# QingzhiWang/LIS-SLAM

Measured on AMD Instinct MI355X. Metric: scan-to-submap registrations/sec (64x1800 pts, 200k submap), higher is better.
Workload: dtype f32; 1 GPU; configs[1]: batch=64 synthetic 64x1800 scans vs one shared 200k-pt submap per GPU, semantic mask off, 10 fixed GN iterations, target index build inside the step; batch_per_gpu=64, submap_points=200000, gn_iters=10, parallelism=independent batches x1 + RCCL all-gather of results

## Files before the change

### lis-slam_amd/csrc/lisreg_api_batch.hip

```cpp
#include "lisreg_batch_plan.hpp"

#include <algorithm>
#include <chrono>
#include <cmath>
#include <cstdio>
#include <cstdlib>
#include <cstring>
#include <string>
#include <vector>

using namespace lisreg;

namespace {

struct CtxTargets {
    const std::vector<Target>& v;
    size_t size() const { return v.size(); }
    TargetView operator()(int slot) const
    {
        const Target& t = v[(size_t)slot];
        return TargetView{ t.valid, { t.n[0], t.n[1] }, { t.n_cells[0], t.n_cells[1] }, { &t.g[0], &t.g[1] }, { t.raw_ptr[0], t.raw_ptr[1] },
                           { t.sorted[0].as<float4>(), t.sorted[1].as<float4>() }, { t.cell_start[0].as<int>(), t.cell_start[1].as<int>() } };
    }
};
// ... 301 lines not shown
    ctx_prof_mark(c, -1);
    return LISREG_OK;
}

void dispatch_order_tables(lisreg_ctx* c, Split split, hipStream_t st)
{
    const auto [o, b] = view(c);
    if (!c->last.xcd_now || (b.live.xcd_cached && split.blk == 0)) return;
    const float4* sorted = b.sort_now ? c->sorted_all.as<float4>() : nullptr;
    const bool by_target = many_targets(o, b);
    int* const pos = c->xcd_tab.as<int>();
    int* const ids = pos + b.n_blocks;
    const int nb0 = split.blk ? split.blk : b.n_blocks;
    launch_xcd_order(c->blocks.as<BlockDesc>(), nb0, c->segs.as<Segment>(), c->grids_dev.as<GridIndex>(), c->items.as<ItemState>(),
                     sorted, by_target, pos, ids, st);
    if (!split.blk) return;
    launch_xcd_order(c->blocks.as<BlockDesc>() + split.blk, b.n_blocks - split.blk, c->segs.as<Segment>(), c->grids_dev.as<GridIndex>(),
                     c->items.as<ItemState>(), sorted, by_target, pos + split.blk, ids + split.blk, st);
    c->batch.live.xcd_cached = false;
}

struct RunHalf { int i0, ni, b0, nb; hipStream_t s; int sidx; hipEvent_t after_assoc; };

void iteration(lisreg_ctx* c, const DevParams& prm, int it, const RunHalf& h)
{
    const auto [o, b] = view(c);
    if (!h.after_assoc) ctx_prof_mark(c, 0, h.sidx);
    (o.exact ? launch_assoc_exact : launch_assoc)(
                 c->blocks.as<BlockDesc>() + h.b0, h.nb, c->segs.as<Segment>(), c->grids_dev.as<GridIndex>(),
                 c->items.as<ItemState>(), prm, b.sort_now ? c->sorted_all.as<float4>() : nullptr, c->partials.as<double>() + (size_t)h.b0 * kNumAcc,
                 b.mode_now, c->nn.as<int>(), b.n_elems, o.first_pass_r * o.first_pass_r,
                 b.mode_now != 5 && it >= (b.lanes_q == 8 ? kWideFromSmall : kWideFrom) && it <= (b.mode_now == 3 ? kGraphWideUntil : kWideUntil), kGraphHops,
                 o.count_searches ? c->counters.as<unsigned long long>() : nullptr,
                 o.dump_neighbors ? c->dbg_nn.as<int>() : nullptr, b.lanes_q,
                 c->blocks_q.as<BlockDesc>(), (int)b.h_blocks_q.size(), c->coef.as<float4>(), c->coef_ok.as<int>(),
                 c->last.xcd_now ? c->xcd_tab.as<int>() + b.n_blocks + h.b0 : nullptr, h.s);
    if (h.after_assoc) (void)hipEventRecord(h.after_assoc, h.s);
    ctx_prof_mark(c, 1, h.sidx);
    launch_solve(c->items.as<ItemState>() + h.i0, h.ni, prm, c->partials.as<double>(),
                 o.trace_cap > 0 ? c->trace.as<float>() + (size_t)h.i0 * (size_t)o.trace_cap * kTraceStride : nullptr, o.trace_cap, c->done_dev.as<int>(), h.s);
    ctx_prof_mark(c, -1, h.sidx);
}

int run_plain(lisreg_ctx* c, const DevParams& prm, bool can_stop, hipStream_t st)
{
    const auto [o, b] = view(c);
    const int chunk = o.early_stop_chunk > 0 ? o.early_stop_chunk : (b.n_blocks <= 1024 ? 6 : 3);
    int next_check = chunk;
    if (o.early_stop_chunk <= 0 && c->mem.last_launches > 0) next_check = std::max(2, std::min(c->mem.last_launches, chunk));
    const RunHalf all{ 0, b.n_items, 0, b.n_blocks, st, 0, nullptr };
    for (int it = 0; it < prm.bound; ++it) {
        iteration(c, prm, it, all);
        if (o.exact && it + 1 < prm.bound) { int rc = exact_pose_caches(c); if (rc) return rc; }
        if (can_stop && it + 1 == next_check && it + 1 < prm.bound) {
            HIPCHK(c, hipMemcpyAsync(c->done_host.p, c->done_dev.p, sizeof(int), hipMemcpyDeviceToHost, st));
            HIPCHK(c, hipStreamSynchronize(st));
            if (*c->done_host.as<int>() >= b.n_items) break;
            next_check += o.early_stop_chunk > 0 ? chunk : std::min(chunk, 3);
        }
    }
    return LISREG_OK;
}

int run_interleaved(lisreg_ctx* c, const DevParams& prm, Split split, hipStream_t st)
{
    const auto [o, b] = view(c);
    c->last.interleaved_now = true;
    const bool alternate = o.interleave == 1 && c->ev_ab && c->ev_ba;
    const RunHalf A{ 0, split.item, 0, split.blk, st, 0, alternate ? (hipEvent_t)c->ev_ab : nullptr };
    const RunHalf B{ split.item, b.n_items - split.item, split.blk, b.n_blocks - split.blk, c->side_stream, 1, alternate ? (hipEvent_t)c->ev_ba : nullptr };
    hipError_t ie = hipSuccess;
    for (int it = 0; it < prm.bound && ie == hipSuccess; ++it) {
        if (alternate && it > 0) ie = hipStreamWaitEvent(st, c->ev_ba, 0);
        if (ie != hipSuccess) break;
        if (alternate) ctx_prof_mark(c, 0, 0);
        iteration(c, prm, it, A);
        if (alternate) ie = hipStreamWaitEvent(c->side_stream, c->ev_ab, 0);
        if (ie != hipSuccess) break;
        if (alternate) ctx_prof_mark(c, 0, 1);
        iteration(c, prm, it, B);
    }
    if (ie == hipSuccess) ie = hipEventRecord(c->ev_join, c->side_stream);
    if (ie == hipSuccess) ie = hipStreamWaitEvent(st, c->ev_join, 0);
    if (ie == hipSuccess) return LISREG_OK;
    (void)hipStreamSynchronize(c->side_stream);
    c->last.interleaved_now = false;
    return ctx_fail(c, LISREG_ERR_HIP, std::string("interleaved run: ") + hipGetErrorString(ie));
}

int finalize_run(lisreg_ctx* c, const DevParams& prm, hipStream_t st)
{
    launch_finalize(c->items.as<ItemState>(), c->batch.n_items, prm, c->results.as<float>(), st, c->done_dev.as<int>());
    c->batch.live.items_reset = true; ++c->batch.live.runs_since_fetch;
    HIPCHK(c, hipGetLastError());
    if (c->pack_in_use >= 0 && c->pack_free[c->pack_in_use])
        HIPCHK(c, hipEventRecord(c->pack_free[c->pack_in_use], st));
    return LISREG_OK;
}

int run_impl(lisreg_ctx* c, bool early_stop)
{
    if (!c->batch.live.prepared) return bad(c, "batch_run: no prepared batch");
    HIPCHK(c, hipSetDevice(c->device));
    const auto [o, b] = view(c);
    PreparedBatch::Live& live = c->batch.live;
    hipStream_t st = c->stream;
    c->last.xcd_now = xcd_order_wanted(o, b);
    if (c->last.xcd_now) HIPCHK(c, c->xcd_tab.ensure(sizeof(int) * 2 * (size_t)b.n_blocks));
    const bool can_stop = early_stop && b.prm.fixed_iters <= 0 && c->done_host.p && o.early_stop_chunk != 0;
    const Split split = choose_split(c, can_stop);
    c->last.reach_now = o.rebuild_targets_each_run && b.mode_now == 5 && live.reach_ready && !o.exact;
    DevParams prm = b.prm;
    prm.reach_miss = c->last.reach_now ? reach_miss_counter(c) : nullptr;
    const bool reset_done = live.items_reset;
    live.items_reset = false;
    if (o.rebuild_targets_each_run) { int rc = rebuild_targets(c, st); if (rc) return rc; }
    if (!reset_done) launch_reset_items(c->items.as<ItemState>(), b.n_items, prm, c->done_dev.as<int>(), st);
    if (o.exact) { int rc = exact_pose_caches(c); if (rc) return rc; }
    ctx_prof_mark(c, 2);
    launch_sort_sources(c->blocks.as<BlockDesc>(), b.n_blocks, c->segs.as<Segment>(), b.n_segs, c->items.as<ItemState>(),
                        b.n_elems, b.sort_now ? b.n_buckets : 0, sort_buffers(c), c->sorted_all.as<float4>(), c->order_all.as<int>(), st);
    ctx_prof_mark(c, -1);
    dispatch_order_tables(c, split, st);
    prm.cell_anchor_until = o.cell_anchor_until;
    c->last.interleaved_now = false;
    int rc;
    if (split.blk > 0 && hipEventRecord(c->ev_fork, st) == hipSuccess && hipStreamWaitEvent(c->side_stream, c->ev_fork, 0) == hipSuccess)
        rc = run_interleaved(c, prm, split, st);
    else
        rc = run_plain(c, prm, can_stop, st);
    return rc ? rc : finalize_run(c, prm, st);
}

using HostClock = std::chrono::steady_clock;
int prepare_run_fetch(lisreg_ctx* c, int n_items, const lisreg_item* dev_items, const lisreg_params* params, float* T, lisreg_stats* stats,
                      const HostClock::time_point* prof)
{
    int rc = lisreg_batch_prepare(c, n_items, dev_items, params, T);
    if (rc) { (void)hipStreamSynchronize(c->stream); return rc; }
    const auto t1 = prof ? HostClock::now() : HostClock::time_point();
    rc = run_impl(c, true);
    if (rc) { (void)hipStreamSynchronize(c->stream); return rc; }
    const auto t2 = prof ? HostClock::now() : HostClock::time_point();
    rc = lisreg_batch_fetch(c, T, stats);
    if (prof) {
        auto us = [](auto a, auto b) { return std::chrono::duration<double, std::micro>(b - a).count(); };
        fprintf(stderr, "[lisreg host] upload %.1f us, prepare %.1f us, enqueue %.1f us, fetch (incl. GPU wait) %.1f us\n",
                us(prof[0], prof[1]), us(prof[1], t1), us(t1, t2), us(t2, HostClock::now()));
    }
    return rc;
}

}

// ... 177 lines not shown
```

### lis-slam_amd/csrc/lisreg_api_ctx.hip

```cpp
#include "lisreg_ctx.hpp"

#include <algorithm>
#include <cmath>
#include <cstring>
#include <string>
#include <vector>

namespace lisreg {

static thread_local std::string g_static_err;
int ctx_fail(lisreg_ctx* c, int code, const std::string& msg)
{
    if (c) c->err = msg; else g_static_err = msg;
    return code;
}

int bad(lisreg_ctx* c, const std::string& msg) { return ctx_fail(c, LISREG_ERR_ARG, msg); }

int check_cloud(lisreg_ctx* c, const char* who, const void* cloud, int n, int stride, int fmt, unsigned accepted_formats, bool allow_empty)
{
    if (n < 0 || (n == 0 && !allow_empty)) return bad(c, std::string(who) + (allow_empty ? ": n < 0" : ": n <= 0"));
    if (n > 0 && !cloud) return bad(c, std::string(who) + ": NULL cloud with n > 0");
    if (fmt < 0 || fmt >= 32 || !(accepted_formats & fmt_bit(fmt))) return bad(c, std::string(who) + ": this fmt is not accepted here");
    if (fmt_bit(fmt) & kFmtDevice) return LISREG_OK;
// ... 115 lines not shown
void make_grid(const float bb_in[6], int n, GridIndex* g, int* n_cells, int margin_cells)
{
    float bb[6] = { bb_in[0], bb_in[1], bb_in[2], bb_in[3], bb_in[4], bb_in[5] };
    memset(g, 0, sizeof *g);
    g->n = n;
    float cell = 0.5f;
    if (n > 0) {
        const double area = std::max(1.0, (double)(bb[3] - bb[0]) * (double)(bb[4] - bb[1]));
        cell = (float)std::min(0.5, std::max(0.25, 2.8 / std::sqrt((double)n / area)));
    }
    if (n <= 0) { g->cell = cell; g->inv_cell = 1.f / cell; g->nx = g->ny = g->nz = 0; *n_cells = 1; return; }
    const double max_cells = 1 << 24;
    const float bb0[6] = { bb[0], bb[1], bb[2], bb[3], bb[4], bb[5] };
    for (;;) {
        for (int d = 0; d < 3; ++d) { bb[d] = bb0[d] - (float)margin_cells * cell; bb[3 + d] = bb0[3 + d] + (float)margin_cells * cell; }
        double nx = floor((bb[3] - bb[0]) / cell) + 1, ny = floor((bb[4] - bb[1]) / cell) + 1,
               nz = floor((bb[5] - bb[2]) / cell) + 1;
        if (nx * ny * nz <= max_cells) { g->nx = (int)nx; g->ny = (int)ny; g->nz = (int)nz; break; }
        cell *= 1.26f;
    }
    g->ox = bb[0]; g->oy = bb[1]; g->oz = bb[2];
    g->cell = cell; g->inv_cell = 1.f / cell;
    *n_cells = g->nx * g->ny * g->nz;
}

}

extern "C" {

const char* lisreg_last_error(const lisreg_ctx* c) { return c ? c->err.c_str() : lisreg::g_static_err.c_str(); }

void lisreg_pose_to_matrix(const float T[6], float M[12])
{
    float A = cosf(T[2]), B = sinf(T[2]), C = cosf(T[1]), D = sinf(T[1]), E = cosf(T[0]), F = sinf(T[0]);
    float DE = D * E, DF = D * F;
    M[0] = A * C;  M[1] = A * DF - B * E;  M[2]  = B * F + A * DE;  M[3]  = T[3];
    M[4] = B * C;  M[5] = A * E + B * DF;  M[6]  = B * DE - A * F;  M[7]  = T[4];
    M[8] = -D;     M[9] = C * F;           M[10] = C * E;           M[11] = T[5];
}

}
```

### lis-slam_amd/csrc/lisreg_assoc.hip

```cpp
#include "lisreg_internal.hpp"

#ifndef LISREG_EXACT
#define LISREG_EXACT 0
#endif
#if LISREG_EXACT
#define LISREG_ASSOC_NS exact_arith
#define LISREG_LAUNCH_ASSOC launch_assoc_exact
#define LISREG_LAUNCH_TEST_FIT launch_test_fit_exact
#else
#define LISREG_ASSOC_NS fast_arith
#define LISREG_LAUNCH_ASSOC launch_assoc
#define LISREG_LAUNCH_TEST_FIT launch_test_fit
#endif

namespace lisreg {

namespace {
namespace LISREG_ASSOC_NS {

constexpr bool kExactArith = LISREG_EXACT != 0;
constexpr int kRedWaveFloats = 1024;
__device__ __forceinline__ float fdiv(float a, float b) { return kExactArith ? a / b : a * __builtin_amdgcn_rcpf(b); }
__device__ __forceinline__ float fsqrt(float x) { return kExactArith ? sqrtf(x) : __builtin_amdgcn_sqrtf(x); }
__device__ __forceinline__ float fdiv5(float a) { return kExactArith ? a / 5.f : a * 0.2f; }
// ... 961 lines not shown
    if (valid) q0 = qsrc[qflat];
    float qx = M[0] * q0.x + M[1] * q0.y + M[2] * q0.z + M[3];
    float qy = M[4] * q0.x + M[5] * q0.y + M[6] * q0.z + M[7];
    float qz = M[8] * q0.x + M[9] * q0.y + M[10] * q0.z + M[11];

    float b0, b1, b2, b3, b4;
    int   i0, i1, i2, i3, i4;
    bool  tie = false;
#define LISREG_LIST_INIT() do { b0 = b1 = b2 = b3 = b4 = P.tau; i0 = i1 = i2 = i3 = i4 = -1; } while (0)
    if (kGraph) {
        bool need_walk = valid, scanned = false;
        if (kGraph == 2) {
            int row_ = -1;
            float mx_ = 0.f, my_ = 0.f, mz_ = 0.f;
            if (valid && g.crow_tab) {
                const float tx = (qx - g.ox) * g.inv_cell, ty = (qy - g.oy) * g.inv_cell, tz = (qz - g.oz) * g.inv_cell;
                const int gx = (int)floorf(tx), gy = (int)floorf(ty), gz = (int)floorf(tz);
                const int hx = min(max(gx, 0), g.nx - 1), hy = min(max(gy, 0), g.ny - 1), hz = min(max(gz, 0), g.nz - 1);
                const int v = ((gptr_i32)g.crow_tab)[(hx * g.ny + hy) * g.nz + hz];
                if (P.reach_miss) {
                    const unsigned long long mm = __ballot(v == -1);
                    if (mm != 0ull && (int)(__ffsll((long long)mm) - 1) == (tid & 63)) atomicAdd(P.reach_miss, __popcll(mm));
                }
                if (v >= 0) {
                    float fx = 0.5f, fy = 0.5f, fz = 0.5f;
                    row_ = v >> 8;
                    {
                        const bool ux = tx - (float)hx >= 0.5f, uy = ty - (float)hy >= 0.5f, uz = tz - (float)hz >= 0.5f;
                        const int oct = (int)ux + 2 * (int)uy + 4 * (int)uz, bit = 1 << oct;
                        if (v & bit) {
                            fx = ux ? 0.75f : 0.25f; fy = uy ? 0.75f : 0.25f; fz = uz ? 0.75f : 0.25f;
                            row_ += 1 + __popc(v & (bit - 1));
                        }
                    }
                    mx_ = crow_centre(g.ox, g.cell, hx, fx); my_ = crow_centre(g.oy, g.cell, hy, fy); mz_ = crow_centre(g.oz, g.cell, hz, fz);
                } else if (v == -2 && hx == gx && hy == gy && hz == gz && P.tau <= (2.f * g.cell - 2.f * kEps) * (2.f * g.cell - 2.f * kEps)) {
                    need_walk = false;
                }
            }
            const gptr_f4 crow = (gptr_f4)g.crow;
            const gptr_f2 cmeta = (gptr_f2)g.crow_meta;
            const bool scan_ = row_ >= 0;
            v2f am_; am_.x = 0.f; am_.y = 0.f;
            if (scan_) am_ = cmeta[row_];
            if (scan_) {
                bool certified = false;
                scanned = true;
                LISREG_CELL_SCAN();
                need_walk = !certified;
            }
        } else
        if (valid && it->iter > 0 && g.nbr) {
            int anchor = nn[qflat];
            if (it->iter <= P.cell_anchor_until) {
                float cd2;
                const int ca = cell_anchor(g, cells, pts, qx, qy, qz, cd2);
                if (ca >= 0) {
                    float od2 = 3.0e38f;
                    if (anchor >= 0) { const v3f ap = LISREG_LD3(pts, anchor); const float x = qx - ap.x, y = qy - ap.y, z = qz - ap.z; od2 = x * x + y * y + z * z; }
                    if (cd2 < od2) anchor = ca;
// ... 358 lines not shown
```

### lis-slam_amd/csrc/lisreg_index.hip

```cpp
#include "lisreg_internal.hpp"

namespace lisreg {

namespace {

constexpr int kScanBlock = 256;
constexpr int kScanItems = 8;
constexpr int kScanTile  = kScanBlock * kScanItems;

__device__ __forceinline__ int wave_incl_scan(int v, int lane)
{
#pragma unroll
    for (int d = 1; d < 64; d <<= 1) {
        int t = __shfl_up(v, d);
        if (lane >= d) v += t;
    }
    return v;
}

__device__ __forceinline__ int block_excl_scan(int v, int* total, int* s_wave )
{
    const int lane = threadIdx.x & 63, wave = threadIdx.x >> 6;
    int inc = wave_incl_scan(v, lane);
    if (lane == 63) s_wave[wave] = inc;
// ... 947 lines not shown
            s_qk[wave][slot] = ck; s_qj[wave][slot] = cj;
        }
        pend += __popcll(m);
        __builtin_amdgcn_wave_barrier();
        if (pend >= 64) {
            const unsigned qk = s_qk[wave][lane]; const int qj = s_qj[wave][lane];
            const int rest = pend - 64;
            unsigned rk = 0u; int rj = 0;
            if (lane < rest) { rk = s_qk[wave][64 + lane]; rj = s_qj[wave][64 + lane]; }
            __builtin_amdgcn_wave_barrier();
            if (lane < rest) { s_qk[wave][lane] = rk; s_qj[wave][lane] = rj; }
            pend = rest;
            __builtin_amdgcn_wave_barrier();
            take(qk, qj, make_float4(0.f, 0.f, 0.f, 0.f));
        }
    }
    if (pend > 0 || first) {
        unsigned qk = kInfQ; int qj = -1;
        if (lane < pend) { qk = s_qk[wave][lane]; qj = s_qj[wave][lane]; }
        take(qk, qj, make_float4(0.f, 0.f, 0.f, 0.f));
    }
}

__device__ __forceinline__ float crow_emit(const GridIndex& g, float qx, float qy, float qz, float rc, unsigned topk, int topi,
                                           float4* __restrict__ row_out, float2* __restrict__ meta_out, bool& keep, float4& e,
                                           const float4 topc = make_float4(0.f, 0.f, 0.f, 0.f), bool have_c = false)
{
    const int lane = threadIdx.x & 63;
    const float tk = __uint_as_float(topk);
    const float dK = __shfl(tk, kGraphK - 1);
    const float rho2 = fminf(rc * rc, dK);
    keep = topi >= 0 && tk <= rho2;
    const int cnt = __popcll(__ballot(keep));
    e = make_float4(qx, qy, qz, __int_as_float(-1));
    if (keep) {
        float4 c = topc;
        if (!have_c) c = g.pts[topi];
        e = make_float4(c.x, c.y, c.z, __int_as_float(topi));
    }
    row_out[lane] = e;
    if (lane == 0) *meta_out = make_float2(rho2, __int_as_float(cnt));
    return rho2;
}

__device__ __forceinline__ void graph_row_q32(const GridIndex& g, const float4 q, int hx, int hy, int hz, int s,
                                              float4* __restrict__ row_out, float2* __restrict__ meta_out, int (*s_off)[64], int (*s_js)[64])
{
    const CrowBlock<2> b = crow_runs<2>(g, hx, hy, hz, s_off, s_js);
    unsigned topk; int topi; float4 topc; bool have_c;
    const float rc = crow_inscribed<2>(g, b, q.x, q.y, q.z);
    crow_list<2, true>(g, b, q.x, q.y, q.z, s_off, s_js, topk, topi, topc, have_c, s, rc * rc);
    bool keep; float4 e;
    (void)crow_emit(g, q.x, q.y, q.z, rc, topk, topi, row_out, meta_out, keep, e, topc, have_c);
}

template <int R>
__device__ __forceinline__ void crow_build_wave(const GridIndex& g, const float4 q, int hx, int hy, int hz, unsigned mask,
                                                float4* __restrict__ row_out, float2* __restrict__ meta_out, int (*s_off)[64], int (*s_js)[64])
{
    const int lane = threadIdx.x & 63;
    constexpr float kEps = 1e-3f;
    const CrowBlock<R> b = crow_runs<R>(g, hx, hy, hz, s_off, s_js);
    unsigned topk; int topi; float4 topc; bool have_c;
    const float rc = crow_inscribed<R>(g, b, q.x, q.y, q.z);
    crow_list<R>(g, b, q.x, q.y, q.z, s_off, s_js, topk, topi, topc, have_c, -1, rc * rc);
    bool keep; float4 e;
    const float rho2 = crow_emit(g, q.x, q.y, q.z, rc, topk, topi, row_out, meta_out, keep, e, topc, have_c);
    if (mask) {
        const float off = 0.25f * g.cell * 1.7320508f;
        const float rho_o = fmaxf(sqrtf(rho2) - off - 2.f * kEps, 0.f), rho_o2 = rho_o * rho_o;
        const bool derive = rho_o >= 1.5f * off;
        int slot = 1;
#pragma unroll 1
        for (int o = 0; o < 8; ++o) {
            if (!((mask >> o) & 1u)) continue;
            const float mx = crow_centre(g.ox, g.cell, hx, o & 1 ? 0.75f : 0.25f), my = crow_centre(g.oy, g.cell, hy, o & 2 ? 0.75f : 0.25f);
            const float mz = crow_centre(g.oz, g.cell, hz, o & 4 ? 0.75f : 0.25f);
            float4* orow = row_out + (size_t)slot * kGraphK;
            if (derive) {
                unsigned k = kInfQ | (unsigned)lane;
                if (keep) {
                    const float ex = mx - e.x, ey = my - e.y, ez = mz - e.z;
                    k = (__float_as_uint(ex * ex + ey * ey + ez * ez) & ~0x7Fu) | (unsigned)lane;
                }
                k = sort64x32(k, lane);
                const int sl = (int)(k & 63u);
                const int oi = __shfl(keep ? topi : -1, sl);
                const float ox = __shfl(e.x, sl), oy = __shfl(e.y, sl), oz = __shfl(e.z, sl);
                const bool okeep = oi >= 0 && __uint_as_float(k & ~0x7Fu) <= rho_o2;
                const int ocnt = __popcll(__ballot(okeep));
                float4 oe = make_float4(mx, my, mz, __int_as_float(-1));
                if (okeep) oe = make_float4(ox, oy, oz, __int_as_float(oi));
                orow[lane] = oe;
                if (lane == 0) meta_out[slot] = make_float2(rho_o2, __int_as_float(ocnt));
            } else {
                unsigned ok; int oi; bool okeep; float4 oe, oc; bool ohave;
                const float orc = crow_inscribed<R>(g, b, mx, my, mz);
                crow_list<R>(g, b, mx, my, mz, s_off, s_js, ok, oi, oc, ohave, -1, orc * orc);
                (void)crow_emit(g, mx, my, mz, orc, ok, oi, orow, meta_out + slot, okeep, oe, oc, ohave);
            }
            ++slot;
        }
    }
}

constexpr int kCrowWPB = 1;
constexpr int kCrowCPW = 8;
constexpr int kCrowWaves = 6;
static_assert(kGraphWPB <= kListQueueWaves && kCrowWPB <= kListQueueWaves, "crow_list's LDS queue has one region per wavefront of a workgroup");
__device__ __forceinline__ void crow_build_body(const GridIndex& g, int n_cells, const int* __restrict__ need, int* __restrict__ omask,
                                                const int* __restrict__ scan, int cap,
                                                int blk_, int (*s_off)[64], int (*s_js)[64])
{
    const int lane = threadIdx.x & 63;
    const int first = __builtin_amdgcn_readfirstlane((blk_ * kCrowWPB + (int)(threadIdx.x >> 6)) * kCrowCPW);
    int* tab = const_cast<int*>(g.crow_tab);
    int n_l = 0, b_l = 0, om_l = 0;
    if (lane < kCrowCPW && first + lane < n_cells) {
        n_l = need[first + lane];
        om_l = omask[first + lane];
        omask[first + lane] = 0;
        if (n_l) b_l = scan[first + lane];
        const bool fits = n_l != 0 && !(b_l + n_l > cap || b_l >= (1 << 23));
        tab[first + lane] = n_l == 0 ? ((om_l & kCrowUnreached) ? -1 : -2) : (fits ? (b_l << 8) | (om_l & 255) : -1);
        if (!fits) n_l = 0;
    }
    unsigned long long live = __ballot(n_l != 0);
#pragma unroll 1
    while (live) {
        const int i = __ffsll((long long)live) - 1;
        live &= live - 1;
        const int cid = first + i;
        const int b = __shfl(b_l, i);
        const unsigned om = (unsigned)__shfl(om_l, i), mask = om & 255u;
        const int hz = cid % g.nz, t = cid / g.nz, hy = t % g.ny, hx = t / g.ny;
        const float4 q = make_float4(crow_centre(g.ox, g.cell, hx, 0.5f), crow_centre(g.oy, g.cell, hy, 0.5f), crow_centre(g.oz, g.cell, hz, 0.5f), 0.f);
        float4* row = const_cast<float4*>(g.crow) + (size_t)b * kGraphK;
        float2* meta = const_cast<float2*>(g.crow_meta) + b;
        if (mask != 0u || (int)(om >> 8) >= kGraphK) crow_build_wave<2>(g, q, hx, hy, hz, mask, row, meta, s_off, s_js);
        else crow_build_wave<3>(g, q, hx, hy, hz, 0u, row, meta, s_off, s_js);
    }
}

__global__ __launch_bounds__(64 * kCrowWPB) __attribute__((amdgpu_waves_per_eu(kCrowWaves, kCrowWaves)))
void k_crow_build(GridIndex g, int n_cells, const int* __restrict__ need, int* __restrict__ omask, const int* __restrict__ scan, int cap)
{
    __shared__ int s_off[kCrowWPB][64], s_js[kCrowWPB][64];
    crow_build_body(g, n_cells, need, omask, scan, cap, blockIdx.x, s_off, s_js);
}

struct CrowJob { GridIndex g; int n_cells; int* need; int* omask; int* scan; int cap; const unsigned* reach; const unsigned* qmark; int tiles_y; int plain; int nb; };
struct CrowJobs { CrowJob j[2]; };
__global__ __launch_bounds__(256) void k_crow_mark_pair(CrowJobs J, float margin_cells)
{
    const int k = (int)blockIdx.x < J.j[0].nb ? 0 : 1;
    const CrowJob& j = J.j[k];
    crow_mark_body(j.g, margin_cells * j.g.cell, j.omask, (int)blockIdx.x - (k ? J.j[0].nb : 0));
}
__global__ __launch_bounds__(256) void k_crow_classify_pair(CrowJobs J, float margin_cells)
{
    extern __shared__ int s_cs[];
    const int k = (int)blockIdx.x < J.j[0].nb ? 0 : 1;
    const CrowJob& j = J.j[k];
    const int blk = (int)blockIdx.x - (k ? J.j[0].nb : 0);
    if (j.plain) crow_classify_plain_body(j.g, j.n_cells, j.need, j.omask, j.reach, j.qmark, blk);
    else crow_classify_body(j.g, j.tiles_y, j.need, j.omask, j.reach, j.qmark, blk, s_cs, margin_cells * j.g.cell);
}
__global__ __launch_bounds__(64 * kCrowWPB) __attribute__((amdgpu_waves_per_eu(kCrowWaves, kCrowWaves))) void k_crow_build_pair(CrowJobs J)
{
    __shared__ int s_off[kCrowWPB][64], s_js[kCrowWPB][64];
    const int k = (int)blockIdx.x < J.j[0].nb ? 0 : 1;
    const CrowJob& j = J.j[k];
    crow_build_body(j.g, j.n_cells, j.need, j.omask, j.scan, j.cap, (int)blockIdx.x - (k ? J.j[0].nb : 0), s_off, s_js);
}

__global__ __launch_bounds__(kBlockQ) void k_count_jumps(const BlockDesc* __restrict__ blocks, const Segment* __restrict__ segs,
                                                         float thr2, int* __restrict__ jumps)
{
    const BlockDesc bd = blocks[blockIdx.x];
    const Segment sg = segs[bd.seg];
    const int e = bd.start + threadIdx.x;
    bool jump = false;
    if ((int)threadIdx.x < bd.count && e + 1 < sg.n) {
        const float4 a = sg.src[e], b = sg.src[e + 1];
        const float dx = a.x - b.x, dy = a.y - b.y, dz = a.z - b.z;
        jump = dx * dx + dy * dy + dz * dz > thr2;
    }
    const unsigned long long m = __ballot(jump);
    if ((threadIdx.x & 63) == 0 && m) atomicAdd(jumps, __popcll(m));
}

__global__ __launch_bounds__(256) void k_voxel_keys(const float4* __restrict__ pts, int n, VoxelDesc d,
                                                    uint32_t* __restrict__ elem_bucket, uint32_t* __restrict__ elem_sub,
                                                    int* __restrict__ hist)
{
    const int i = blockIdx.x * 256 + threadIdx.x;
// ... 622 lines not shown
```

### lis-slam_amd/csrc/lisreg_internal.hpp

```cpp
#pragma once
#include <hip/hip_runtime.h>
#include <stdint.h>
#include "../../include/lisreg.h"

namespace lisreg {

constexpr int kBlockQ     = 256;
constexpr int kNumAcc     = 28;
constexpr int kResultSize = 12;
constexpr int kTraceStride = LISREG_TRACE_STRIDE;
constexpr int kGraphK     = 64;

struct GridIndex {
    const float4* pts;
    const int*    cell_start;
    int   n;
    float ox, oy, oz;
    float cell, inv_cell;
    int   nx, ny, nz;
    const float4* nbr;
    const float2* nbr_meta;
    const float4* crow;
    const float2* crow_meta;
    const int*    crow_tab;
    unsigned*     qmark;
    int           qmark_w;
};


__device__ __forceinline__ float crow_centre(float origin, float cell, int h, float off) { return __builtin_fmaf((float)h + off, cell, origin); }

struct Segment {
    const float4* src;
    int   n;
    int   item;
    int   kind;
    int   target;
    int   flat_base;
    int   bucket_base;
    int   tnx, tny, tnz;
    float tox, toy, toz;
    float inv_tile;
};

struct TargetSeg {
    const float4* raw;
    float4*       sorted_out;
    int*          cell_start_out;
    int   n, n_cells;
// ... 113 lines not shown
                  const ItemState* items, DevParams prm, const float4* sorted_all, double* partials,
                  int mode ,
                  int* nn, int n_elems, float first_pass_r2,
                  bool wide ,
                  int graph_hops ,
                  unsigned long long* counters ,
                  int* dbg_nn ,
                  int lanes_q ,
                  const BlockDesc* blocks_q, int n_blocks_q ,
                  float4* coef, int* coef_ok ,
                  const int* xcd_order , hipStream_t st);
void launch_assoc_exact(const BlockDesc* blocks, int n_blocks, const Segment* segs, const GridIndex* grids,
                        const ItemState* items, DevParams prm, const float4* sorted_all, double* partials,
                        int mode, int* nn, int n_elems, float first_pass_r2, bool wide, int graph_hops,
                        unsigned long long* counters, int* dbg_nn, int lanes_q, const BlockDesc* blocks_q, int n_blocks_q,
                        float4* coef, int* coef_ok, const int* xcd_order, hipStream_t st);
void launch_test_fit(int kind, int n, const float* nb15, const float* q3, DevParams prm, float* out, hipStream_t st);
void launch_test_fit_exact(int kind, int n, const float* nb15, const float* q3, DevParams prm, float* out, hipStream_t st);
void launch_xcd_order(const BlockDesc* blocks, int n_blocks, const Segment* segs, const GridIndex* grids, const ItemState* items,
                      const float4* sorted_all, bool by_target, int* keys, int* order, hipStream_t st);
void launch_pose_gather(const ItemState* items, int n_items, float* T_out, hipStream_t st);
void launch_pose_cache_from_trig(ItemState* items, int n_items, const float* trig, hipStream_t st);
void launch_solve(ItemState* items, int n_items, DevParams prm, const double* partials, float* trace,
                  int trace_cap, int* done_counter, hipStream_t st);
void launch_finalize(ItemState* items, int n_items, DevParams prm, float* results, hipStream_t st, int* reset_done_counter = nullptr);

void launch_voxel_sort(const float4* pts, int n, VoxelDesc d, int n_buckets, SortBuffers sb, int* order, uint32_t* sidx,
                       int* head, int* slot , hipStream_t st);
void launch_voxel_starts(int n, const int* head, const int* slot, int* vstart , hipStream_t st);
struct VoxelHandOut { int k; int vo[kVoxelMultiMax + 1]; float4* out[kVoxelMultiMax]; };
void launch_bbox_multi(const float4* cat, const VoxelMulti& m, float* bbox_out , float* scratch , hipStream_t st);
struct BboxJobs { int k; int n[kVoxelMultiMax]; const float4* pts[kVoxelMultiMax]; };
void launch_bbox_jobs(const BboxJobs& j, float* bbox_out , float* scratch , hipStream_t st);
struct CloudRef { const float4* pts; int n; int pad_; };
void launch_bbox_refs(const CloudRef* refs_dev, int k, float* bbox_out , float* scratch , hipStream_t st);
void launch_concat_jobs(const BboxJobs& j, const VoxelMulti& m, float4* cat, hipStream_t st);
void launch_multi_bounds(const int* slot, const VoxelMulti& m, int* out , hipStream_t st);
void launch_hand_out(const float4* src, const VoxelHandOut& h, hipStream_t st);
void launch_voxel_sort_multi(const float4* pts, int n, const VoxelMulti& m, int n_buckets, SortBuffers sb, int* order, uint32_t* sidx,
                             int* head, int* slot, hipStream_t st);
void launch_voxel_centroids(int n, int n_vox, const float4* pts, const uint32_t* labels, int w_mode, const int* order,
                            const int* head, const int* slot, int* vstart , float4* out_pts,
                            uint32_t* out_labels , hipStream_t st);
void launch_pack_cloud(const void* raw_dev, size_t n, int stride, int has_label, float4* out, hipStream_t st);
void launch_transform_cloud(const float4* in, int n, const float* M12_dev, float4* out, hipStream_t st);
struct Mat12 { float m[12]; };
__device__ __forceinline__ float4 transform_record(const float4 p, const float* __restrict__ M12)
// ... 88 lines not shown
```

### lis-slam_amd/csrc/lisreg_solve.hip

```cpp
#include "lisreg_internal.hpp"

namespace lisreg {

namespace {

__device__ float hyp(float a, float b)
{
    a = fabsf(a); b = fabsf(b);
    if (a > b) { b /= a; return a * sqrtf(1.f + b * b); }
    if (b > 0.f) { a /= b; return b * sqrtf(1.f + a * a); }
    return 0.f;
}

__device__ void eigen_sym6(float* A, float* W, float* V, int* indR, int* indC)
{
    const int n = 6;
    for (int i = 0; i < n; ++i) for (int j = 0; j < n; ++j) V[i * n + j] = (i == j) ? 1.f : 0.f;
    for (int k = 0; k < n; ++k) {
        W[k] = A[k * n + k];
        if (k < n - 1) {
            int m = k + 1; float mv = fabsf(A[k * n + m]);
            for (int i = k + 2; i < n; ++i) { float v = fabsf(A[k * n + i]); if (mv < v) { mv = v; m = i; } }
            indR[k] = m;
        }
// ... 165 lines not shown
    const bool guard_ok = (it->n_sc > P.edge_min) && (it->n_ss > P.surf_min);
    it->iter = 0;
    it->guard_failed = guard_ok ? 0 : 1;
    it->done = guard_ok ? 0 : 1;
    it->iters_out = 0;
    it->deltaR = 100.f; it->deltaT = 100.f;
    it->degenerate = it->degenerate_in;
    it->n_corr = 0;
    it->any_solved = 0;
    write_pose_cache(it);
}

__global__ __launch_bounds__(64) void k_reset_items(ItemState* __restrict__ items, int n_items, const DevParams P,
                                                    int* __restrict__ done_counter, int* __restrict__ zero_too)
{
    const int i = blockIdx.x * 64 + threadIdx.x;
    if (i == 0) { *done_counter = P.n_guard_failed; if (zero_too) *zero_too = 0; }
    if (i >= n_items) return;
    reset_item(&items[i], P);
}

constexpr int kSolveThreads = 512;

__global__ __launch_bounds__(kSolveThreads) void k_solve(ItemState* __restrict__ items, const DevParams P,
                                                         const double* __restrict__ partials,
                                                         float* __restrict__ trace, int trace_cap,
                                                         int* __restrict__ done_counter)
{
    __shared__ float s_AtA[36], s_AtB[6], s_X[6], s_A[36];
    __shared__ float s_E[6], s_V[36], s_V2[36], s_Vi[36];
    __shared__ int   s_ind[12];
    __shared__ double s_part[kSolveThreads / 32][32];
    __shared__ double s_sum[kNumAcc];
    __shared__ double s_L[36];

    ItemState* it = &items[blockIdx.x];
    if (it->done) return;
    {
        const int col = threadIdx.x & 31, grp = threadIdx.x >> 5;
        double s = 0.0;
        if (col < kNumAcc) {
            const double* p = partials + (size_t)it->blk_begin * kNumAcc + col;
            const int nb = it->blk_count;
            constexpr int kG = kSolveThreads / 32;
            for (int b = grp; b < nb; b += 32 * kG) {
                double v[32];
#pragma unroll
                for (int u = 0; u < 32; ++u) v[u] = (b + u * kG < nb) ? p[(size_t)(b + u * kG) * kNumAcc] : 0.0;
#pragma unroll
                for (int u = 0; u < 32; ++u) s += v[u];
            }
        }
        s_part[grp][col] = s;
    }
    __syncthreads();
    if (threadIdx.x < kNumAcc) {
        double s = 0.0;
#pragma unroll
        for (int g = 0; g < kSolveThreads / 32; ++g) s += s_part[g][threadIdx.x];
        s_sum[threadIdx.x] = s;
// ... 90 lines not shown
        if (l0) write_pose_cache(it, trig);
        if (l0) {
            const double r0 = (double)(s_X[0] * 57.29578f), r1 = (double)(s_X[1] * 57.29578f), r2 = (double)(s_X[2] * 57.29578f);
            const double t0 = (double)(s_X[3] * 100.f), t1 = (double)(s_X[4] * 100.f), t2 = (double)(s_X[5] * 100.f);
            const float dR = (float)sqrt(r0 * r0 + r1 * r1 + r2 * r2);
            const float dT = (float)sqrt(t0 * t0 + t1 * t1 + t2 * t2);
            it->deltaR = dR; it->deltaT = dT;
            it->degenerate = isDeg;
            it->any_solved = 1;
            if (tr) {
                for (int i = 0; i < 36; ++i) tr[1 + i] = s_AtA[i];
                for (int i = 0; i < 6; ++i) { tr[37 + i] = s_AtB[i]; tr[43 + i] = s_X[i]; tr[49 + i] = it->T[i]; }
                tr[55] = 1.f;
            }
            if (dR < P.conv_deg && dT < P.conv_cm && P.fixed_iters <= 0) {
                it->iters_out = iter;
                finished = true;
            }
        }
    }
    if (l0) {
        it->iter = iter + 1;
        if (!finished && iter + 1 >= P.bound) { it->iters_out = P.bound; finished = true; }
        if (finished) { it->done = 1; atomicAdd(done_counter, 1); }
    }
}

struct Quat { double x, y, z, w; };
__device__ Quat q_rpy(double roll, double pitch, double yaw)
{
    const double hy = yaw * 0.5, hp = pitch * 0.5, hr = roll * 0.5;
    const double cy = cos(hy), sy = sin(hy), cp = cos(hp), sp = sin(hp), cr = cos(hr), sr = sin(hr);
    return Quat{ sr * cp * cy - cr * sp * sy, cr * sp * cy + sr * cp * sy, cr * cp * sy - sr * sp * cy,
                 cr * cp * cy + sr * sp * sy };
}
__device__ double q_dot(Quat a, Quat b) { return a.x * b.x + a.y * b.y + a.z * b.z + a.w * b.w; }
__device__ Quat q_slerp(Quat a, Quat b, double t)
{
    const double s = sqrt(q_dot(a, a) * q_dot(b, b));
    const double d = q_dot(a, b);
    const double theta = (d < 0 ? acos(-d / s) * 2.0 : acos(d / s) * 2.0) / 2.0;
    if (theta != 0.0) {
        const double dd = 1.0 / sin(theta), s0 = sin((1.0 - t) * theta), s1 = sin(t * theta);
        const double sg = d < 0 ? -1.0 : 1.0;
        return Quat{ (a.x * s0 + sg * b.x * s1) * dd, (a.y * s0 + sg * b.y * s1) * dd,
                     (a.z * s0 + sg * b.z * s1) * dd, (a.w * s0 + sg * b.w * s1) * dd };
    }
// ... 5 lines not shown
    const double xs = q.x * s, ys = q.y * s, zs = q.z * s;
    const double wx = q.w * xs, wy = q.w * ys, wz = q.w * zs;
    const double xx = q.x * xs, xy = q.x * ys, xz = q.x * zs, yy = q.y * ys, yz = q.y * zs, zz = q.z * zs;
    const double m00 = 1.0 - (yy + zz), m10 = xy + wz, m20 = xz - wy, m21 = yz + wx, m22 = 1.0 - (xx + yy);
    if (fabs(m20) >= 1) {
        yaw = 0;
        roll = atan2(m21, m22);
        pitch = m20 < 0 ? 1.5707963267948966 : -1.5707963267948966;
    } else {
        pitch = -asin(m20);
        const double cp = cos(pitch);
        roll = atan2(m21 / cp, m22 / cp);
        yaw = atan2(m10 / cp, m00 / cp);
    }
}
__device__ float clampf(float v, float lim) { v = v < -lim ? -lim : v; return v > lim ? lim : v; }

__global__ __launch_bounds__(64) void k_finalize(ItemState* __restrict__ items, int n_items, const DevParams P,
                                                 float* __restrict__ results, int* __restrict__ reset_done_counter)
{
    const int i = blockIdx.x * 64 + threadIdx.x;
    if (i == 0 && reset_done_counter) *reset_done_counter = P.n_guard_failed;
    if (i >= n_items) return;
    ItemState* it = &items[i];
    float T[6];
    for (int k = 0; k < 6; ++k) T[k] = it->T[k];
    int status = LISREG_OK;
    if (it->guard_failed) status = LISREG_NOT_ENOUGH_FEATURES;
    else {
        if (P.use_imu && it->imu.imu_available && fabsf(it->imu.imu_pitch_init) < 1.4f) {
            const double w = (double)P.imu_w;
            double r, p, y;
            q_get_rpy(q_slerp(q_rpy((double)T[0], 0, 0), q_rpy((double)it->imu.imu_roll_init, 0, 0), w), r, p, y);
            T[0] = (float)r;
            q_get_rpy(q_slerp(q_rpy(0, (double)T[1], 0), q_rpy(0, (double)it->imu.imu_pitch_init, 0), w), r, p, y);
            T[1] = (float)p;
        }
        T[0] = clampf(T[0], P.rot_tol);
        T[1] = clampf(T[1], P.rot_tol);
        T[5] = clampf(T[5], P.z_tol);
        if (!it->any_solved) status = LISREG_TOO_FEW_CORRESPONDENCES;
    }
    float* r = results + (size_t)i * kResultSize;
    for (int k = 0; k < 6; ++k) r[k] = T[k];
    r[6] = (float)it->iters_out; r[7] = it->deltaR; r[8] = it->deltaT;
    r[9] = (float)it->degenerate; r[10] = (float)it->n_corr; r[11] = (float)status;
    if (reset_done_counter) reset_item(it, P);
}

__global__ __launch_bounds__(64) void k_pose_gather(const ItemState* __restrict__ items, int n_items, float* __restrict__ T_out)
{
    const int i = blockIdx.x * 64 + threadIdx.x;
    if (i >= n_items) return;
    for (int k = 0; k < 6; ++k) T_out[6 * i + k] = items[i].T[k];
}
__global__ __launch_bounds__(64) void k_pose_cache_from_trig(ItemState* __restrict__ items, int n_items, const float* __restrict__ trig)
{
    const int i = blockIdx.x * 64 + threadIdx.x;
    if (i >= n_items) return;
    write_pose_cache(&items[i], trig + 6 * i);
}

}

void launch_pose_gather(const ItemState* items, int n_items, float* T_out, hipStream_t st)
{
    if (n_items > 0) k_pose_gather<<<(n_items + 63) / 64, 64, 0, st>>>(items, n_items, T_out);
}
void launch_pose_cache_from_trig(ItemState* items, int n_items, const float* trig, hipStream_t st)
{
    if (n_items > 0) k_pose_cache_from_trig<<<(n_items + 63) / 64, 64, 0, st>>>(items, n_items, trig);
}

void launch_reset_items(ItemState* items, int n_items, DevParams prm, int* done_counter, hipStream_t st, int* zero_too)
{
    k_reset_items<<<(std::max(n_items, 1) + 63) / 64, 64, 0, st>>>(items, n_items, prm, done_counter, zero_too);
}

void launch_solve(ItemState* items, int n_items, DevParams prm, const double* partials, float* trace,
                  int trace_cap, int* done_counter, hipStream_t st)
{
    if (n_items > 0) k_solve<<<n_items, kSolveThreads, 0, st>>>(items, prm, partials, trace, trace_cap, done_counter);
}

void launch_finalize(ItemState* items, int n_items, DevParams prm, float* results, hipStream_t st, int* reset_done_counter)
{
    if (n_items > 0) k_finalize<<<(n_items + 63) / 64, 64, 0, st>>>(items, n_items, prm, results, reset_done_counter);
}

}
```

Baseline: 30940 registrations/s.

## Fuse finalize into last solve, prune empty cells via grid margin, trim crow stores

Three independent changes. With fixed iterations and no early stop, the last GN solve launch writes the results and resets items itself, so the separate finalize kernel is no longer launched. The grid now records a margin between the point bounding box and the padded grid, and association uses it (plus a ring-distance bound for empty cells) to skip the neighbour walk when no point can lie within tau. The fused crow builder also stops writing row slots beyond the rounded-up count of kept entries. Together these target launch overhead, wasted walk work and memory writes, at the cost of a more delicate done-counter reset and looser pruning bounds that must stay correct.

```diff
diff --git a/lis-slam_amd/csrc/lisreg_api_batch.hip b/lis-slam_amd/csrc/lisreg_api_batch.hip
--- a/lis-slam_amd/csrc/lisreg_api_batch.hip
+++ b/lis-slam_amd/csrc/lisreg_api_batch.hip
@@ -347,7 +347,7 @@
 
 struct RunHalf { int i0, ni, b0, nb; hipStream_t s; int sidx; hipEvent_t after_assoc; };
 
-void iteration(lisreg_ctx* c, const DevParams& prm, int it, const RunHalf& h)
+void iteration(lisreg_ctx* c, const DevParams& prm, int it, const RunHalf& h, float* results_of_last_launch = nullptr)
 {
     const auto [o, b] = view(c);
     if (!h.after_assoc) ctx_prof_mark(c, 0, h.sidx);
@@ -363,19 +363,23 @@
     if (h.after_assoc) (void)hipEventRecord(h.after_assoc, h.s);
     ctx_prof_mark(c, 1, h.sidx);
     launch_solve(c->items.as<ItemState>() + h.i0, h.ni, prm, c->partials.as<double>(),
-                 o.trace_cap > 0 ? c->trace.as<float>() + (size_t)h.i0 * (size_t)o.trace_cap * kTraceStride : nullptr, o.trace_cap, c->done_dev.as<int>(), h.s);
+                 o.trace_cap > 0 ? c->trace.as<float>() + (size_t)h.i0 * (size_t)o.trace_cap * kTraceStride : nullptr, o.trace_cap, c->done_dev.as<int>(), h.s,
+                 results_of_last_launch);
     ctx_prof_mark(c, -1, h.sidx);
 }
 
-int run_plain(lisreg_ctx* c, const DevParams& prm, bool can_stop, hipStream_t st)
+int run_plain(lisreg_ctx* c, const DevParams& prm, bool can_stop, hipStream_t st, bool* finalized)
 {
     const auto [o, b] = view(c);
     const int chunk = o.early_stop_chunk > 0 ? o.early_stop_chunk : (b.n_blocks <= 1024 ? 6 : 3);
     int next_check = chunk;
     if (o.early_stop_chunk <= 0 && c->mem.last_launches > 0) next_check = std::max(2, std::min(c->mem.last_launches, chunk));
     const RunHalf all{ 0, b.n_items, 0, b.n_blocks, st, 0, nullptr };
+    const bool fuse = !can_stop && !o.exact && prm.fixed_iters > 0 && b.n_items > 0;
     for (int it = 0; it < prm.bound; ++it) {
-        iteration(c, prm, it, all);
+        const bool last = fuse && it + 1 == prm.bound;
+        iteration(c, prm, it, all, last ? c->results.as<float>() : nullptr);
+        if (last) *finalized = true;
         if (o.exact && it + 1 < prm.bound) { int rc = exact_pose_caches(c); if (rc) return rc; }
         if (can_stop && it + 1 == next_check && it + 1 < prm.bound) {
             HIPCHK(c, hipMemcpyAsync(c->done_host.p, c->done_dev.p, sizeof(int), hipMemcpyDeviceToHost, st));
@@ -413,9 +417,9 @@
     return ctx_fail(c, LISREG_ERR_HIP, std::string("interleaved run: ") + hipGetErrorString(ie));
 }
 
-int finalize_run(lisreg_ctx* c, const DevParams& prm, hipStream_t st)
-{
-    launch_finalize(c->items.as<ItemState>(), c->batch.n_items, prm, c->results.as<float>(), st, c->done_dev.as<int>());
+int finalize_run(lisreg_ctx* c, const DevParams& prm, hipStream_t st, bool finalized)
+{
+    if (!finalized) launch_finalize(c->items.as<ItemState>(), c->batch.n_items, prm, c->results.as<float>(), st, c->done_dev.as<int>());
     c->batch.live.items_reset = true; ++c->batch.live.runs_since_fetch;
     HIPCHK(c, hipGetLastError());
     if (c->pack_in_use >= 0 && c->pack_free[c->pack_in_use])
@@ -450,11 +454,12 @@
     prm.cell_anchor_until = o.cell_anchor_until;
     c->last.interleaved_now = false;
     int rc;
+    bool finalized = false;
     if (split.blk > 0 && hipEventRecord(c->ev_fork, st) == hipSuccess && hipStreamWaitEvent(c->side_stream, c->ev_fork, 0) == hipSuccess)
         rc = run_interleaved(c, prm, split, st);
     else
-        rc = run_plain(c, prm, can_stop, st);
-    return rc ? rc : finalize_run(c, prm, st);
+        rc = run_plain(c, prm, can_stop, st, &finalized);
+    return rc ? rc : finalize_run(c, prm, st, finalized);
 }
 
 using HostClock = std::chrono::steady_clock;
diff --git a/lis-slam_amd/csrc/lisreg_api_ctx.hip b/lis-slam_amd/csrc/lisreg_api_ctx.hip
--- a/lis-slam_amd/csrc/lisreg_api_ctx.hip
+++ b/lis-slam_amd/csrc/lisreg_api_ctx.hip
@@ -161,6 +161,15 @@
     g->ox = bb[0]; g->oy = bb[1]; g->oz = bb[2];
     g->cell = cell; g->inv_cell = 1.f / cell;
     *n_cells = g->nx * g->ny * g->nz;
+    if (margin_cells > 0) {
+        const int dims[3] = { g->nx, g->ny, g->nz };
+        double m = (double)margin_cells * cell;
+        for (int d = 0; d < 3; ++d) {
+            m = std::min(m, (double)bb0[d] - (double)bb[d]);
+            m = std::min(m, (double)fmaf((float)dims[d], cell, bb[d]) - (double)bb0[3 + d]);
+        }
+        g->margin = (float)std::max(m, 0.0);
+    }
 }
 
 }
diff --git a/lis-slam_amd/csrc/lisreg_assoc.hip b/lis-slam_amd/csrc/lisreg_assoc.hip
--- a/lis-slam_amd/csrc/lisreg_assoc.hip
+++ b/lis-slam_amd/csrc/lisreg_assoc.hip
@@ -1007,7 +1007,29 @@
                     const unsigned long long mm = __ballot(v == -1);
                     if (mm != 0ull && (int)(__ffsll((long long)mm) - 1) == (tid & 63)) atomicAdd(P.reach_miss, __popcll(mm));
                 }
-                if (v >= 0) {
+                bool empty_ = false;
+                if (hx != gx || hy != gy || hz != gz) {
+                    const float ex_ = gx < 0 ? g.ox - qx : qx - __builtin_fmaf((float)g.nx, g.cell, g.ox);
+                    const float ey_ = gy < 0 ? g.oy - qy : qy - __builtin_fmaf((float)g.ny, g.cell, g.oy);
+                    const float ez_ = gz < 0 ? g.oz - qz : qz - __builtin_fmaf((float)g.nz, g.cell, g.oz);
+                    const float lx_ = hx != gx ? fmaxf(ex_ + g.margin - kEps, 0.f) : 0.f;
+                    const float ly_ = hy != gy ? fmaxf(ey_ + g.margin - kEps, 0.f) : 0.f;
+                    const float lz_ = hz != gz ? fmaxf(ez_ + g.margin - kEps, 0.f) : 0.f;
+                    empty_ = lx_ * lx_ + ly_ * ly_ + lz_ * lz_ >= P.tau;
+                } else if (v == -2) {
+                    float rc_ = 3.0e18f;
+                    if (hx - 2 > 0)        rc_ = fminf(rc_, qx - (g.ox + (float)(hx - 2) * g.cell));
+                    if (hx + 2 < g.nx - 1) rc_ = fminf(rc_, (g.ox + (float)(hx + 3) * g.cell) - qx);
+                    if (hy - 2 > 0)        rc_ = fminf(rc_, qy - (g.oy + (float)(hy - 2) * g.cell));
+                    if (hy + 2 < g.ny - 1) rc_ = fminf(rc_, (g.oy + (float)(hy + 3) * g.cell) - qy);
+                    if (hz - 2 > 0)        rc_ = fminf(rc_, qz - (g.oz + (float)(hz - 2) * g.cell));
+                    if (hz + 2 < g.nz - 1) rc_ = fminf(rc_, (g.oz + (float)(hz + 3) * g.cell) - qz);
+                    rc_ = fmaxf(rc_ - kEps, 0.f);
+                    empty_ = rc_ * rc_ >= P.tau;
+                }
+                if (empty_) {
+                    need_walk = false;
+                } else if (v >= 0) {
                     float fx = 0.5f, fy = 0.5f, fz = 0.5f;
                     row_ = v >> 8;
                     {
@@ -1019,8 +1041,6 @@
                         }
                     }
                     mx_ = crow_centre(g.ox, g.cell, hx, fx); my_ = crow_centre(g.oy, g.cell, hy, fy); mz_ = crow_centre(g.oz, g.cell, hz, fz);
-                } else if (v == -2 && hx == gx && hy == gy && hz == gz && P.tau <= (2.f * g.cell - 2.f * kEps) * (2.f * g.cell - 2.f * kEps)) {
-                    need_walk = false;
                 }
             }
             const gptr_f4 crow = (gptr_f4)g.crow;
diff --git a/lis-slam_amd/csrc/lisreg_index.hip b/lis-slam_amd/csrc/lisreg_index.hip
--- a/lis-slam_amd/csrc/lisreg_index.hip
+++ b/lis-slam_amd/csrc/lisreg_index.hip
@@ -993,9 +993,10 @@
     }
 }
 
+template <bool kTrim = false>
 __device__ __forceinline__ float crow_emit(const GridIndex& g, float qx, float qy, float qz, float rc, unsigned topk, int topi,
                                            float4* __restrict__ row_out, float2* __restrict__ meta_out, bool& keep, float4& e,
-                                           const float4 topc = make_float4(0.f, 0.f, 0.f, 0.f), bool have_c = false)
+                                           const float4 topc = make_float4(0.f, 0.f, 0.f, 0.f), bool have_c = false, bool store = true)
 {
     const int lane = threadIdx.x & 63;
     const float tk = __uint_as_float(topk);
@@ -1009,7 +1010,7 @@
         if (!have_c) c = g.pts[topi];
         e = make_float4(c.x, c.y, c.z, __int_as_float(topi));
     }
-    row_out[lane] = e;
+    if (kTrim ? (store && lane < ((cnt + 3) & ~3)) : true) row_out[lane] = e;
     if (lane == 0) *meta_out = make_float2(rho2, __int_as_float(cnt));
     return rho2;
 }
@@ -1025,7 +1026,7 @@
     (void)crow_emit(g, q.x, q.y, q.z, rc, topk, topi, row_out, meta_out, keep, e, topc, have_c);
 }
 
-template <int R>
+template <int R, bool kTrim>
 __device__ __forceinline__ void crow_build_wave(const GridIndex& g, const float4 q, int hx, int hy, int hz, unsigned mask,
                                                 float4* __restrict__ row_out, float2* __restrict__ meta_out, int (*s_off)[64], int (*s_js)[64])
 {
@@ -1036,7 +1037,7 @@
     const float rc = crow_inscribed<R>(g, b, q.x, q.y, q.z);
     crow_list<R>(g, b, q.x, q.y, q.z, s_off, s_js, topk, topi, topc, have_c, -1, rc * rc);
     bool keep; float4 e;
-    const float rho2 = crow_emit(g, q.x, q.y, q.z, rc, topk, topi, row_out, meta_out, keep, e, topc, have_c);
+    const float rho2 = crow_emit<kTrim>(g, q.x, q.y, q.z, rc, topk, topi, row_out, meta_out, keep, e, topc, have_c, mask != 255u);
     if (mask) {
         const float off = 0.25f * g.cell * 1.7320508f;
         const float rho_o = fmaxf(sqrtf(rho2) - off - 2.f * kEps, 0.f), rho_o2 = rho_o * rho_o;
@@ -1062,13 +1063,13 @@
                 const int ocnt = __popcll(__ballot(okeep));
                 float4 oe = make_float4(mx, my, mz, __int_as_float(-1));
                 if (okeep) oe = make_float4(ox, oy, oz, __int_as_float(oi));
-                orow[lane] = oe;
+                if (!kTrim || lane < ((ocnt + 3) & ~3)) orow[lane] = oe;
                 if (lane == 0) meta_out[slot] = make_float2(rho_o2, __int_as_float(ocnt));
             } else {
                 unsigned ok; int oi; bool okeep; float4 oe, oc; bool ohave;
                 const float orc = crow_inscribed<R>(g, b, mx, my, mz);
                 crow_list<R>(g, b, mx, my, mz, s_off, s_js, ok, oi, oc, ohave, -1, orc * orc);
-                (void)crow_emit(g, mx, my, mz, orc, ok, oi, orow, meta_out + slot, okeep, oe, oc, ohave);
+                (void)crow_emit<kTrim>(g, mx, my, mz, orc, ok, oi, orow, meta_out + slot, okeep, oe, oc, ohave);
             }
             ++slot;
         }
@@ -1079,6 +1080,7 @@
 constexpr int kCrowCPW = 8;
 constexpr int kCrowWaves = 6;
 static_assert(kGraphWPB <= kListQueueWaves && kCrowWPB <= kListQueueWaves, "crow_list's LDS queue has one region per wavefront of a workgroup");
+template <bool kTrim>
 __device__ __forceinline__ void crow_build_body(const GridIndex& g, int n_cells, const int* __restrict__ need, int* __restrict__ omask,
                                                 const int* __restrict__ scan, int cap,
                                                 int blk_, int (*s_off)[64], int (*s_js)[64])
@@ -1108,8 +1110,8 @@
         const float4 q = make_float4(crow_centre(g.ox, g.cell, hx, 0.5f), crow_centre(g.oy, g.cell, hy, 0.5f), crow_centre(g.oz, g.cell, hz, 0.5f), 0.f);
         float4* row = const_cast<float4*>(g.crow) + (size_t)b * kGraphK;
         float2* meta = const_cast<float2*>(g.crow_meta) + b;
-        if (mask != 0u || (int)(om >> 8) >= kGraphK) crow_build_wave<2>(g, q, hx, hy, hz, mask, row, meta, s_off, s_js);
-        else crow_build_wave<3>(g, q, hx, hy, hz, 0u, row, meta, s_off, s_js);
+        if (mask != 0u || (int)(om >> 8) >= kGraphK) crow_build_wave<2, kTrim>(g, q, hx, hy, hz, mask, row, meta, s_off, s_js);
+        else crow_build_wave<3, kTrim>(g, q, hx, hy, hz, 0u, row, meta, s_off, s_js);
     }
 }
 
@@ -1117,7 +1119,7 @@
 void k_crow_build(GridIndex g, int n_cells, const int* __restrict__ need, int* __restrict__ omask, const int* __restrict__ scan, int cap)
 {
     __shared__ int s_off[kCrowWPB][64], s_js[kCrowWPB][64];
-    crow_build_body(g, n_cells, need, omask, scan, cap, blockIdx.x, s_off, s_js);
+    crow_build_body<false>(g, n_cells, need, omask, scan, cap, blockIdx.x, s_off, s_js);
 }
 
 struct CrowJob { GridIndex g; int n_cells; int* need; int* omask; int* scan; int cap; const unsigned* reach; const unsigned* qmark; int tiles_y; int plain; int nb; };
@@ -1142,7 +1144,7 @@
     __shared__ int s_off[kCrowWPB][64], s_js[kCrowWPB][64];
     const int k = (int)blockIdx.x < J.j[0].nb ? 0 : 1;
     const CrowJob& j = J.j[k];
-    crow_build_body(j.g, j.n_cells, j.need, j.omask, j.scan, j.cap, (int)blockIdx.x - (k ? J.j[0].nb : 0), s_off, s_js);
+    crow_build_body<true>(j.g, j.n_cells, j.need, j.omask, j.scan, j.cap, (int)blockIdx.x - (k ? J.j[0].nb : 0), s_off, s_js);
 }
 
 __global__ __launch_bounds__(kBlockQ) void k_count_jumps(const BlockDesc* __restrict__ blocks, const Segment* __restrict__ segs,
diff --git a/lis-slam_amd/csrc/lisreg_internal.hpp b/lis-slam_amd/csrc/lisreg_internal.hpp
--- a/lis-slam_amd/csrc/lisreg_internal.hpp
+++ b/lis-slam_amd/csrc/lisreg_internal.hpp
@@ -25,6 +25,7 @@
     const int*    crow_tab;
     unsigned*     qmark;
     int           qmark_w;
+    float         margin;
 };
 
 
@@ -184,7 +185,7 @@
 void launch_pose_gather(const ItemState* items, int n_items, float* T_out, hipStream_t st);
 void launch_pose_cache_from_trig(ItemState* items, int n_items, const float* trig, hipStream_t st);
 void launch_solve(ItemState* items, int n_items, DevParams prm, const double* partials, float* trace,
-                  int trace_cap, int* done_counter, hipStream_t st);
+                  int trace_cap, int* done_counter, hipStream_t st, float* results_of_last_launch = nullptr);
 void launch_finalize(ItemState* items, int n_items, DevParams prm, float* results, hipStream_t st, int* reset_done_counter = nullptr);
 
 void launch_voxel_sort(const float4* pts, int n, VoxelDesc d, int n_buckets, SortBuffers sb, int* order, uint32_t* sidx,
diff --git a/lis-slam_amd/csrc/lisreg_solve.hip b/lis-slam_amd/csrc/lisreg_solve.hip
--- a/lis-slam_amd/csrc/lisreg_solve.hip
+++ b/lis-slam_amd/csrc/lisreg_solve.hip
@@ -211,10 +211,12 @@
 
 constexpr int kSolveThreads = 512;
 
+__device__ void finalize_item(ItemState* it, const DevParams& P, float* __restrict__ r, bool reset);
+
 __global__ __launch_bounds__(kSolveThreads) void k_solve(ItemState* __restrict__ items, const DevParams P,
                                                          const double* __restrict__ partials,
                                                          float* __restrict__ trace, int trace_cap,
-                                                         int* __restrict__ done_counter)
+                                                         int* __restrict__ done_counter, float* __restrict__ results)
 {
     __shared__ float s_AtA[36], s_AtB[6], s_X[6], s_A[36];
     __shared__ float s_E[6], s_V[36], s_V2[36], s_Vi[36];
@@ -224,7 +226,11 @@
     __shared__ double s_L[36];
 
     ItemState* it = &items[blockIdx.x];
-    if (it->done) return;
+    float* const res = results ? results + (size_t)blockIdx.x * kResultSize : nullptr;
+    if (it->done) {
+        if (res && threadIdx.x == 0) finalize_item(it, P, res, true);
+        return;
+    }
     {
         const int col = threadIdx.x & 31, grp = threadIdx.x >> 5;
         double s = 0.0;
@@ -361,7 +367,12 @@
     if (l0) {
         it->iter = iter + 1;
         if (!finished && iter + 1 >= P.bound) { it->iters_out = P.bound; finished = true; }
-        if (finished) { it->done = 1; atomicAdd(done_counter, 1); }
+        if (finished) {
+            it->done = 1;
+            const int before = atomicAdd(done_counter, 1);
+            if (res && before + 1 == (int)gridDim.x) atomicExch(done_counter, P.n_guard_failed);
+        }
+        if (res) finalize_item(it, P, res, true);
     }
 }
 
@@ -413,7 +424,11 @@
     const int i = blockIdx.x * 64 + threadIdx.x;
     if (i == 0 && reset_done_counter) *reset_done_counter = P.n_guard_failed;
     if (i >= n_items) return;
-    ItemState* it = &items[i];
+    finalize_item(&items[i], P, results + (size_t)i * kResultSize, reset_done_counter != nullptr);
+}
+
+__device__ void finalize_item(ItemState* it, const DevParams& P, float* __restrict__ r, bool reset)
+{
     float T[6];
     for (int k = 0; k < 6; ++k) T[k] = it->T[k];
     int status = LISREG_OK;
@@ -432,11 +447,10 @@
         T[5] = clampf(T[5], P.z_tol);
         if (!it->any_solved) status = LISREG_TOO_FEW_CORRESPONDENCES;
     }
-    float* r = results + (size_t)i * kResultSize;
     for (int k = 0; k < 6; ++k) r[k] = T[k];
     r[6] = (float)it->iters_out; r[7] = it->deltaR; r[8] = it->deltaT;
     r[9] = (float)it->degenerate; r[10] = (float)it->n_corr; r[11] = (float)status;
-    if (reset_done_counter) reset_item(it, P);
+    if (reset) reset_item(it, P);
 }
 
 __global__ __launch_bounds__(64) void k_pose_gather(const ItemState* __restrict__ items, int n_items, float* __restrict__ T_out)
@@ -469,9 +483,9 @@
 }
 
 void launch_solve(ItemState* items, int n_items, DevParams prm, const double* partials, float* trace,
-                  int trace_cap, int* done_counter, hipStream_t st)
-{
-    if (n_items > 0) k_solve<<<n_items, kSolveThreads, 0, st>>>(items, prm, partials, trace, trace_cap, done_counter);
+                  int trace_cap, int* done_counter, hipStream_t st, float* results_of_last_launch)
+{
+    if (n_items > 0) k_solve<<<n_items, kSolveThreads, 0, st>>>(items, prm, partials, trace, trace_cap, done_counter, results_of_last_launch);
 }
 
 void launch_finalize(ItemState* items, int n_items, DevParams prm, float* results, hipStream_t st, int* reset_done_counter)
```

Result: no change. 31230 registrations/s (median of 6 runs) (+0.9%).
